# RIVM-bioinformatics/TrueConsense

Measured on NVIDIA B200. Metric: aligned_bases_per_sec_pileup_consensus, higher is better.
Workload: dtype int32

## Files before the change

### trueconsense_b200/csrc/cuda/inserts.cu

```cuda
#include <cub/device/device_segmented_radix_sort.cuh>

#include <memory>
#include <new>

#include "tc_common.cuh"

constexpr int INS_TILE = 256;
constexpr uint64_t KEY_NONE = ~0ull;
constexpr int INS_TBL = 4096;
constexpr int INS_BASES_FIXED = 64;

struct ins_args {
    dreads r;
    const int32_t* cand;
    int n_cand;
    const int32_t* n_cand_dev;
    uint32_t flag_filter; int min_mapq, min_bq, ignore_orphans; long long max_depth;
    int32_t span_hint;
    int32_t* range;
    uint32_t* range_off;
    const int64_t* seg_off;
    const int32_t* tile_cand;
    const int32_t* tile_first;
    int32_t* tile_sel;
    int32_t* tile_last;
    uint64_t* ent_key; int32_t* ent_indel; int32_t* ent_qpos; uint8_t* ent_head;
    uint8_t* ent_sel;
    uint8_t* ent_q;
    uint8_t* pair_q; unsigned long long pair_cap; unsigned long long* pair_bump;
    int olap_mode;
    int32_t* seg_count;
    int32_t* pair_any;
    int32_t* overflow;
    const int32_t* layout;
    uint8_t* bases_fixed;
    tc_status* status;
};

__device__ __forceinline__ int ins_ncand(const ins_args& a) { return a.n_cand_dev ? min(*a.n_cand_dev, a.n_cand) : a.n_cand; }

__global__ void max_span_kernel(dreads r, tc_status* status) {
    int64_t i = (int64_t)blockIdx.x * blockDim.x + threadIdx.x;
    int span = 0;
    if (i < r.n) {
        if (i > 0 && r.pos[i] < r.pos[i - 1]) atomicCAS(&status->err, 0, TC_ERR_UNSORTED);
        for (uint32_t k = r.cigar_off[i]; k < r.cigar_off[i + 1]; ++k) {
            uint32_t c = r.cigar[k];
            if (op_consumes_ref(c & 15u)) span += (int)(c >> 4);
        }
    }
    span = __reduce_max_sync(0xffffffffu, span);
    if ((threadIdx.x & 31) == 0 && span > 0) atomicMax(&status->max_span, span);
}

// ... 1 lines not shown
    int64_t lo = 0, hi = n;
    while (hi > lo) {
        const int64_t step = (hi - lo + 31) / 32;
        const int64_t i = lo + (int64_t)lane * step;
        const bool ge = i >= hi || pos[i] >= v;
        const unsigned m = __ballot_sync(0xffffffffu, ge);
        if (m == 0u) { lo = lo + 31 * step + 1; continue; }
        const int first = __ffs(m) - 1;
        if (first == 0) return (int)lo;
        hi = min(hi, lo + (int64_t)first * step);
        lo = lo + (int64_t)(first - 1) * step + 1;
    }
    return (int)lo;
}

__global__ void cand_range_kernel(ins_args a) {
    const int ci = blockIdx.x * (blockDim.x >> 5) + (threadIdx.x >> 5);
    const int lane = threadIdx.x & 31;
    if (ci >= ins_ncand(a)) return;
    const int c = a.cand[ci] - 1;
    const int ms = max(a.span_hint > 0 ? a.span_hint : a.status->max_span, 1);
    const int lo = warp_lower_bound(a.r.pos, a.r.n, c - ms + 1, lane);
    const int hi = max(lo, warp_lower_bound(a.r.pos, a.r.n, c + 1, lane));
    if (lane == 0) {
        a.range[2 * ci] = lo;
        a.range[2 * ci + 1] = hi;
        a.range_off[4 * ci] = a.r.seq_off[lo]; a.range_off[4 * ci + 1] = a.r.seq_off[hi];
        a.range_off[4 * ci + 2] = a.r.cigar_off[lo]; a.range_off[4 * ci + 3] = a.r.cigar_off[hi];
    }
}

__device__ __forceinline__ uint64_t mix_key(uint64_t h, uint64_t v) {
    h ^= v + 0x9e3779b97f4a7c15ull + (h << 6) + (h >> 2);
    h *= 0xff51afd7ed558ccdull;
    h ^= h >> 33;
    return h;
}

// ... 52 lines not shown
    for (int t = threadIdx.x; t < n_tiles_s; t += blockDim.x) {
        int lo = 0, hi = n_cand - 1;
        while (lo < hi) { const int mid = (lo + hi + 1) >> 1; if (tile_first[mid] <= t) lo = mid; else hi = mid - 1; }
        tile_cand[t] = lo;
    }
}

__global__ void __launch_bounds__(INS_TILE) ins_select_kernel(ins_args a) {
    __shared__ int wlast[INS_TILE / 32];
    const int tile = blockIdx.x;
    if (a.layout && tile >= a.layout[0]) return;
    const int ci = a.tile_cand[tile];
    const int c = a.cand[ci] - 1;
    const int lo = a.range[2 * ci], hi = a.range[2 * ci + 1];
    const int r = lo + (tile - a.tile_first[ci]) * INS_TILE + threadIdx.x;
    bool sel = false, emit = false, proper = false;
    if (r < hi) {
        const int pos = a.r.pos[r];
        if (r > 0 && pos < a.r.pos[r - 1]) atomicCAS(&a.status->err, 0, TC_ERR_UNSORTED);
        const uint32_t fl = a.r.flag[r];
        const bool pass = !(fl & (a.flag_filter | 4u)) && !(a.min_mapq > 0 && a.r.mapq && (int)a.r.mapq[r] < a.min_mapq) &&
                          !(a.ignore_orphans && (fl & 1u) && !(fl & 2u));
        int indel = 0, qpos = 0, qv = 0; char head = 0; uint64_t key = KEY_NONE;
        if (pass) {
            const uint32_t c0 = a.r.cigar_off[r];
            const int n = (int)(a.r.cigar_off[r + 1] - c0);
            const uint32_t* cig = a.r.cigar + c0;
            const bool rev = (fl & 16u) != 0;
            const int lq = a.r.l_seq[r];
            int x = pos, y = 0;
            bool found = false;
            for (int k = 0; k < n; ++k) {
                const uint32_t cc = cig[k]; const uint32_t op = cc & 15u; const int l = (int)(cc >> 4);
                if (!op_consumes_ref(op)) { if (op == OP_I || op == OP_S) y += l; continue; }
                if (c < x + l) {
                    found = true;
                    const bool match = op_is_match(op);
                    qpos = match ? y + (c - x) : y;
                    if (c == x + l - 1) indel = peek_indel(cig, n, k);
                    qv = (qpos < lq) ? (int)a.r.qual[8ull * a.r.seq_off[r] + qpos] : 0;
                    if (qv >= a.min_bq || a.min_bq > 0) {
                        emit = true;
                        if (match) head = (qpos < lq) ? base_char_upper(seq_code(a.r.seq4 + a.r.seq_off[r], qpos), rev) : 'N';
                        else head = (op == OP_N) ? (rev ? '<' : '>') : '*';
                    }
                    break;
                }
                if (op_is_match(op)) y += l;
                x += l;
            }
            sel = found || (x == pos && pos == c);
            if (emit) {
                const read_syms rs = read_syms_of(a, r);
                bool exact = false;
                if (indel <= 8 && indel > -8192) {
                    exact = true;
                    key = (1ull << 62) | ((uint64_t)((uint8_t)head & 127u) << 54) | ((uint64_t)(uint32_t)(indel + 8192) << 40);
                    for (int j = 1; j <= indel; ++j) key |= (uint64_t)rs.sym(qpos + j) << (5 * (j - 1));
                } else if (indel <= 12) {
                    exact = true;
                    key = (3ull << 61) | ((uint64_t)((uint8_t)head & 127u) << 54) | ((uint64_t)(uint32_t)indel << 48);
                    for (int j = 1; j <= indel; ++j) {
                        const uint32_t sy = rs.sym(qpos + j);
                        exact = exact && sy < 16u;
// ... 15 lines not shown
        proper = sel && (fl & 2u);
    }
    if (__syncthreads_or(proper) && threadIdx.x == 0) a.pair_any[ci] = 1;
    const int nsel = __syncthreads_count(sel);
    int last = __reduce_max_sync(0xffffffffu, sel ? r : -1);
    if ((threadIdx.x & 31) == 0) wlast[threadIdx.x >> 5] = last;
    __syncthreads();
    if (threadIdx.x == 0) {
#pragma unroll
        for (int w = 0; w < INS_TILE / 32; ++w) last = max(last, wlast[w]);
        a.tile_sel[tile] = nsel;
        a.tile_last[tile] = last;
    }
}

__global__ void __launch_bounds__(INS_TILE) ins_admit_kernel(ins_args a) {
    __shared__ int wsum[INS_TILE / 32], wlast[INS_TILE / 32];
    __shared__ long long base_s;
    __shared__ int prev_s;
    const int tile = blockIdx.x;
    if (a.layout && tile >= a.layout[0]) return;
    const int ci = a.tile_cand[tile];
    const int lo = a.range[2 * ci], hi = a.range[2 * ci + 1];
    const int t0 = a.tile_first[ci];
    const int lane = threadIdx.x & 31, warp = threadIdx.x >> 5;
    if (warp == 0) {
        long long base = 0; int prev = -1;
        for (int t = t0 + lane; t < tile; t += 32) { base += a.tile_sel[t]; prev = max(prev, a.tile_last[t]); }
#pragma unroll
        for (int o = 16; o; o >>= 1) { base += __shfl_xor_sync(0xffffffffu, base, o); prev = max(prev, __shfl_xor_sync(0xffffffffu, prev, o)); }
// ... 8 lines not shown
#pragma unroll
    for (int o = 1; o < 32; o <<= 1) { const int t = __shfl_up_sync(0xffffffffu, m, o); if (lane >= o) m = max(m, t); }
    int prev = __shfl_up_sync(0xffffffffu, m, 1);
    if (lane == 0) prev = -1;
    if (lane == 31) wlast[warp] = m;
    if (lane == 0) wsum[warp] = __popc(bal);
    __syncthreads();
    long long rank = base_s + __popc(bal & ((1u << lane) - 1));
    prev = max(prev, prev_s);
    for (int w = 0; w < warp; ++w) { rank += wsum[w]; prev = max(prev, wlast[w]); }
    bool admitted = false;
    if (sel) {
        const bool first_at_start = prev < 0 || a.r.pos[prev] != a.r.pos[r];
        admitted = first_at_start || rank < a.max_depth;
    }
    if (a.min_bq > 0) {
        if (r < hi && admitted) a.ent_sel[slot] = (uint8_t)(es | 4);
        return;
    }
    if (emit && !admitted) a.ent_key[slot] = KEY_NONE;
    const int n_adm = __syncthreads_count(emit && admitted);
    if (threadIdx.x == 0 && n_adm) atomicAdd(&a.seg_count[ci], n_adm);
}

__device__ __forceinline__ uint32_t wang_hash(uint32_t key) {
    key += ~(key << 15); key ^= (key >> 10); key += (key << 3); key ^= (key >> 6); key += ~(key << 11); key ^= (key >> 16);
    return key;
}

struct cwalk { const uint32_t* cig; const uint32_t* end; long long icig, iseq, iref; };

__device__ int iref2iseq_set(cwalk& w, long long pos) {
    if (pos < 0) return -1;
    w.icig = 0; w.iseq = 0; w.iref = 0;
    while (w.cig < w.end) {
        const uint32_t cig = *w.cig & 15u; const long long ncig = (long long)(*w.cig >> 4);
        if (cig == OP_S) { w.cig++; w.iseq += ncig; w.icig = 0; continue; }
// ... 98 lines not shown
        for (uint32_t k = a.r.cigar_off[r]; k < a.r.cigar_off[r + 1]; ++k) { const uint32_t c = a.r.cigar[k]; if (op_consumes_ref(c & 15u)) end += (int)(c >> 4); }
        if (mp >= end) return false;
    }
    return true;
}

__global__ void __launch_bounds__(1024) ins_pair_kernel(ins_args a) {
    extern __shared__ __align__(16) unsigned char pair_smem[];
    unsigned int* tmin = reinterpret_cast<unsigned int*>(pair_smem);
    unsigned int* tmax = tmin + PAIR_TBL;
    unsigned short* tcnt = reinterpret_cast<unsigned short*>(tmax + PAIR_TBL);
    __shared__ int over_s, nadm_s;
    const int ci = blockIdx.x;
    if (ci >= ins_ncand(a)) return;
    if (a.layout && a.layout[2]) return;
    const int64_t off = a.seg_off[ci];
    const int lo = a.range[2 * ci];
    const int n = a.range[2 * ci + 1] - lo;
    const bool pairing = a.olap_mode != 1 && a.r.qname_hash && a.r.mpos && a.r.isize && a.pair_any[ci];
    if (threadIdx.x == 0) { over_s = 0; nadm_s = 0; }
    if (pairing) {
        for (int i = threadIdx.x; i < PAIR_TBL; i += blockDim.x) { tmin[i] = 0u; tmax[i] = 0u; tcnt[i] = 0; }
        __syncthreads();
        auto is_event = [&](int i, bool& push) -> bool {
            const uint8_t es = a.ent_sel[off + i];
            if (!(es & 1)) return false;
            if (!(es & 4)) { push = false; return true; }
            push = true;
            return true;
        };
        for (int pass = 0; pass < 2; ++pass) {
            for (int i = threadIdx.x; i < n; i += blockDim.x) {
                bool push;
                if (!is_event(i, push) || push != (pass == 0)) continue;
                const uint32_t r = (uint32_t)(lo + i);
                if (push && !(a.r.flag[r] & 2u)) continue;
                const unsigned long long k = a.r.qname_hash[r];
                unsigned h = (unsigned)(k ^ (k >> 31)) & (PAIR_TBL - 1);
                int probes = 0;
                for (;;) {
                    const unsigned cur = push ? atomicCAS(&tmin[h], 0u, (unsigned)i + 1u) : tmin[h];
                    if (cur == 0u && !push) break;
                    if (cur == 0u || a.r.qname_hash[lo + cur - 1] == k) {
                        atomicMin(&tmin[h], (unsigned)i + 1u); atomicMax(&tmax[h], (unsigned)i + 1u);
                        atomicAdd(reinterpret_cast<unsigned int*>(tcnt) + (h >> 1), (h & 1) ? 0x10000u : 1u);
                        break;
                    }
                    h = (h + 1) & (PAIR_TBL - 1);
                    if (++probes >= PAIR_TBL * 3 / 4) { over_s = 1; break; }
                }
            }
            __syncthreads();
        }
        __syncthreads();
        if (over_s) { if (threadIdx.x == 0) atomicCAS(&a.status->err, 0, TC_ERR_CAPACITY); return; }
        for (int h = threadIdx.x; h < PAIR_TBL; h += blockDim.x) {
            const int cnt = tcnt[h];
            if (cnt < 2) continue;
            const int first = (int)tmin[h] - 1, last = (int)tmax[h] - 1;
            const unsigned long long k = a.r.qname_hash[lo + first];
            int stored = -1;
            int seen = 0;
            for (int i = first; i <= last && seen < cnt; i = (cnt == 2 && i == first) ? last : i + 1) {
                bool push;
                if (!is_event(i, push)) continue;
                const uint32_t r = (uint32_t)(lo + i);
                if (a.r.qname_hash[r] != k || (push && !(a.r.flag[r] & 2u))) continue;
                ++seen;
                if (!push) { stored = -1; continue; }
                if (!olap_eligible(a, r)) continue;
                bool has_span = false;
                for (uint32_t q = a.r.cigar_off[r]; q < a.r.cigar_off[r + 1] && !has_span; ++q) { const uint32_t c = a.r.cigar[q]; has_span = op_consumes_ref(c & 15u) && (c >> 4) > 0; }
                if (!has_span) continue;
                if (stored < 0) {
                    const int mp = a.r.mpos[r];
                    if (mp >= a.r.pos[r] || ((a.r.flag[r] & 1u) && mp == -1)) stored = i;
                    continue;
                }
                const int64_t sa = off + stored, sb = off + i;
                const uint32_t ra = (uint32_t)(lo + stored);
                const int la = a.r.l_seq[ra], lb = a.r.l_seq[r];
                const unsigned long long at = atomicAdd(a.pair_bump, (unsigned long long)(la + lb));
                if (at + (unsigned long long)(la + lb) <= a.pair_cap) {
                    uint8_t* aq = a.pair_q + at; uint8_t* bq = aq + la;
                    const uint8_t* ga = a.r.qual + 8ull * a.r.seq_off[ra]; const uint8_t* gb = a.r.qual + 8ull * a.r.seq_off[r];
                    for (int q = 0; q < la; ++q) aq[q] = ga[q];
                    for (int q = 0; q < lb; ++q) bq[q] = gb[q];
                    tweak_pair(a, ra, r, aq, bq, a.olap_mode);
                    if ((a.ent_sel[sa] & 2) && a.ent_qpos[sa] < la) a.ent_q[sa] = aq[a.ent_qpos[sa]];
                    if ((a.ent_sel[sb] & 2) && a.ent_qpos[sb] < lb) a.ent_q[sb] = bq[a.ent_qpos[sb]];
                } else atomicOr(a.overflow, 2);
                stored = -1;
            }
        }
        __syncthreads();
    }
    int mine = 0;
    for (int i = threadIdx.x; i < n; i += blockDim.x) {
        const uint8_t es = a.ent_sel[off + i];
        const bool ok = (es & 6) == 6 && (int)a.ent_q[off + i] >= a.min_bq;
        if (!ok) a.ent_key[off + i] = KEY_NONE;
        mine += ok ? 1 : 0;
    }
    mine = __reduce_add_sync(0xffffffffu, mine);
    if ((threadIdx.x & 31) == 0 && mine) atomicAdd(&nadm_s, mine);
    __syncthreads();
    if (threadIdx.x == 0) a.seg_count[ci] = nadm_s;
}

__device__ __forceinline__ bool same_entry(const ins_args& a, int lo, int64_t off, uint32_t e1, uint32_t e2) {
    if (a.ent_head[e1] != a.ent_head[e2] || a.ent_indel[e1] != a.ent_indel[e2]) return false;
    const int indel = a.ent_indel[e1];
    if (indel <= 0) return true;
    const read_syms s1 = read_syms_of(a, (uint32_t)(lo + (int64_t)e1 - off)), s2 = read_syms_of(a, (uint32_t)(lo + (int64_t)e2 - off));
    const int q1 = a.ent_qpos[e1], q2 = a.ent_qpos[e2];
    for (int j = 1; j <= indel; ++j)
        if (s1.sym(q1 + j) != s2.sym(q2 + j)) return false;
// ... 15 lines not shown
        const uint32_t e = (uint32_t)off + (uint32_t)(0xffffffffull - (best & 0xffffffffull));
        out.mode_count = (int32_t)(best >> 32);
        out.first_read = (int32_t)(a.range[2 * ci] + (int64_t)e - off);
        out.head = a.ent_head[e];
        out.indel = a.ent_indel[e];
        out.bases_off = (int64_t)e;
        if (out.indel > 0 && out.indel <= INS_BASES_FIXED) {
            const read_syms rs = read_syms_of(a, (uint32_t)out.first_read);
            const int q = a.ent_qpos[e];
            for (int j = 1; j <= out.indel; ++j) a.bases_fixed[(size_t)ci * INS_BASES_FIXED + j - 1] = sym_char(rs.sym(q + j));
        }
    }
    calls[ci] = out;
}

__global__ void __launch_bounds__(1024) ins_count_kernel(ins_args a, tc_insert_call_t* __restrict__ calls) {
    extern __shared__ __align__(16) unsigned char ins_smem[];
    unsigned long long* tkey = reinterpret_cast<unsigned long long*>(ins_smem);
    unsigned int* tcnt = reinterpret_cast<unsigned int*>(tkey + INS_TBL);
    unsigned int* tfirst = tcnt + INS_TBL;
    __shared__ unsigned long long best_s;
    __shared__ int over_s, hashed_s;
    const int ci = blockIdx.x;
    if (ci >= ins_ncand(a)) return;
    if (a.layout && a.layout[2]) return;
    const int64_t off = a.seg_off[ci];
    const int lo = a.range[2 * ci];
    const int n = a.range[2 * ci + 1] - lo;
    for (int i = threadIdx.x; i < INS_TBL; i += blockDim.x) { tkey[i] = KEY_NONE; tcnt[i] = 0; tfirst[i] = 0xffffffffu; }
    if (threadIdx.x == 0) { best_s = 0ull; over_s = 0; hashed_s = 0; }
    __syncthreads();
    for (int base = 0; base < n; base += 4 * (int)blockDim.x) {
        unsigned long long kk[4];
#pragma unroll
        for (int u = 0; u < 4; ++u) {
            const int i = base + u * (int)blockDim.x + (int)threadIdx.x;
            kk[u] = i < n ? a.ent_key[off + i] : KEY_NONE;
        }
#pragma unroll
        for (int u = 0; u < 4; ++u) {
            const int i = base + u * (int)blockDim.x + (int)threadIdx.x;
            const unsigned long long k = kk[u];
            const unsigned grp = __match_any_sync(0xffffffffu, k);
            if (k == KEY_NONE || (__ffs(grp) - 1) != (int)(threadIdx.x & 31)) continue;
            if (!(k >> 62)) hashed_s = 1;
            unsigned h = (unsigned)(k ^ (k >> 29)) & (INS_TBL - 1);
            int probes = 0;
            for (;;) {
                const unsigned long long old = atomicCAS(&tkey[h], KEY_NONE, k);
                if (old == KEY_NONE || old == k) { atomicAdd(&tcnt[h], (unsigned)__popc(grp)); atomicMin(&tfirst[h], (unsigned)i); break; }
                h = (h + 1) & (INS_TBL - 1);
                if (++probes >= INS_TBL * 7 / 8) { over_s = 1; break; }
            }
        }
    }
    __syncthreads();
    if (over_s) { if (threadIdx.x == 0) atomicOr(a.overflow, 1); return; }
    if (hashed_s)
    for (int i = threadIdx.x; i < n; i += blockDim.x) {
        const unsigned long long k = a.ent_key[off + i];
        if (k == KEY_NONE || (k >> 62)) continue;
        unsigned h = (unsigned)(k ^ (k >> 29)) & (INS_TBL - 1);
        while (tkey[h] != k) h = (h + 1) & (INS_TBL - 1);
        const unsigned f = tfirst[h];
        if (f != (unsigned)i && !same_entry(a, lo, off, (uint32_t)(off + f), (uint32_t)(off + i))) atomicCAS(&a.status->err, 0, TC_ERR_RANGE);
    }
    unsigned long long best = 0ull;
    for (int i = threadIdx.x; i < INS_TBL; i += blockDim.x)
        if (tcnt[i]) best = max(best, ((unsigned long long)tcnt[i] << 32) | (0xffffffffull - (unsigned long long)tfirst[i]));
    atomicMax(&best_s, best);
    __syncthreads();
    if (threadIdx.x == 0) write_call(a, ci, a.seg_count[ci], best_s, calls);
}

__global__ void __launch_bounds__(1024) ins_mode_kernel(ins_args a, const uint64_t* __restrict__ skey, const uint32_t* __restrict__ sidx,
                                                        tc_insert_call_t* __restrict__ calls) {
    __shared__ unsigned long long best_s;
    const int ci = blockIdx.x;
    const int64_t off = a.seg_off[ci];
    const int lo_read = a.range[2 * ci];
    const int m = a.seg_count[ci];
    if (threadIdx.x == 0) best_s = 0ull;
    __syncthreads();
    unsigned long long best = 0ull;
    for (int i = threadIdx.x; i < m; i += blockDim.x) {
        const uint64_t k = skey[off + i];
        int lo = 0, hi = i;
// ... 31 lines not shown
    for (int j = threadIdx.x; j < c.indel; j += blockDim.x) bases[c.bases_off + j] = (uint8_t)ins_char(a, r, a.ent_qpos[e], j + 1, rev);
}

static ins_block ins_block_of(int n_cand, bool with_extra) {
    static_assert(sizeof(tc_status) <= 64, "tc_status outgrew its place in the results block");
    ins_block b;
    b.layout = 64; b.over = 80; b.bump = 88;
    b.extra = with_extra ? 128 : 0;
    b.seg = with_extra ? b.extra + 4 * (TC_RB_EXTRA_CAND + (size_t)n_cand) : 96;
    b.calls = b.seg + ((4 * (2 * (size_t)n_cand + 2) + 15) & ~(size_t)15);
    b.fixed = b.calls + sizeof(tc_insert_call_t) * (size_t)n_cand;
    b.bytes = b.fixed + (size_t)n_cand * INS_BASES_FIXED;
    return b;
}

static int ins_bind(tc_ctx* ctx, ins_args& a, uint8_t* d_rb, const ins_block& rb, size_t T, size_t NT, int n_cand, const tc_pileup_params_t* p) {
    const size_t bytes = T * (8 + 4 + 4 + 1 + 1 + 1) + NT * 12 + ((size_t)n_cand + 1) * 16 + 256 + 16;
    uint8_t* slab = (uint8_t*)tc_dev_buf(ctx, SLOT_INS_D, bytes);
    if (!slab) return TC_ERR_NOMEM;
    a.ent_key = (uint64_t*)slab;
    int64_t* d_off = (int64_t*)(a.ent_key + T);
    a.seg_off = d_off;
    a.ent_indel = (int32_t*)(d_off + n_cand + 1); a.ent_qpos = a.ent_indel + T;
    int32_t* d_tcand = a.ent_qpos + T; int32_t* d_tfirst = d_tcand + NT;
    a.tile_cand = d_tcand; a.tile_first = d_tfirst;
    a.tile_sel = d_tfirst + n_cand + 1; a.tile_last = a.tile_sel + NT;
    a.ent_head = (uint8_t*)(a.tile_last + NT); a.ent_sel = a.ent_head + T; a.ent_q = a.ent_sel + T;
    a.seg_count = (int32_t*)(d_rb + rb.seg); a.pair_any = a.seg_count + n_cand + 1; a.overflow = (int32_t*)(d_rb + rb.over);
    a.bases_fixed = d_rb + rb.fixed;
    if (ctx->pair_cap <= 0) ctx->pair_cap = 1 << 22;
    a.pair_bump = (unsigned long long*)(d_rb + rb.bump); a.pair_cap = (unsigned long long)ctx->pair_cap;
    a.pair_q = (uint8_t*)tc_dev_buf(ctx, SLOT_INS_F, (size_t)ctx->pair_cap);
    if (!a.pair_q) return TC_ERR_NOMEM;
    a.flag_filter = p->flag_filter; a.min_mapq = p->min_mapq; a.min_bq = p->min_base_quality; a.ignore_orphans = p->ignore_orphans;
    a.olap_mode = (p->reserved >> 8) & 3;
// ... 16 lines not shown
        ins_select_kernel<<<tiles, INS_TILE, 0, s>>>(a);
        TC_LAUNCH_CHECK();
        ins_admit_kernel<<<tiles, INS_TILE, 0, s>>>(a);
        TC_LAUNCH_CHECK();
    }
    if (a.min_bq > 0) {
        const size_t smem = (size_t)PAIR_TBL * 10;
        if (!(ctx->ins_attr_set & 2)) {
            TC_CUDA(cudaFuncSetAttribute(ins_pair_kernel, cudaFuncAttributeMaxDynamicSharedMemorySize, (int)smem));
            ctx->ins_attr_set |= 2;
        }
        ins_pair_kernel<<<grid, 1024, smem, s>>>(a);
        TC_LAUNCH_CHECK();
    }
    if (d_calls) {
        const size_t smem = (size_t)INS_TBL * 16;
        if (!(ctx->ins_attr_set & 1)) {
            TC_CUDA(cudaFuncSetAttribute(ins_count_kernel, cudaFuncAttributeMaxDynamicSharedMemorySize, (int)smem));
            ctx->ins_attr_set |= 1;
        }
        ins_count_kernel<<<grid, 1024, smem, s>>>(a, d_calls);
        TC_LAUNCH_CHECK();
    }
    return TC_OK;
}

static int ins_check_status(tc_ctx* ctx, const tc_status& st) {
    if (st.err == TC_ERR_UNSORTED) return tc_fail(ctx, TC_ERR_UNSORTED, "Unsorted input. Pileup aborts");
    if (st.err) return tc_fail(ctx, st.err, "insertion key collision or device-side failure %d", st.err);
    return TC_OK;
}

static int ins_place_bases(tc_ctx* ctx, tc_insert_call_t* calls, int n, const uint8_t* fixed, uint8_t* bases, int64_t bases_cap,
                           int64_t* need_out = nullptr) {
    int64_t need = 0;
    for (int i = 0; i < n; ++i) {
// ... 42 lines not shown
    if (!ctx) return TC_ERR_ARG;
    if (!reads || !p || (n_cand > 0 && (!cand_pos || !calls)) || n_cand < 0 || ref_len <= 0) return tc_fail(ctx, TC_ERR_ARG, "bad argument");
    if (n_cand == 0) return TC_OK;
    if (tc_is_device_ptr(cand_pos) || tc_is_device_ptr(calls) || (bases && tc_is_device_ptr(bases)))
        return tc_fail(ctx, TC_ERR_ARG, "tc_extract_inserts takes host pointers for cand_pos / calls / bases");
    for (int i = 0; i < n_cand; ++i)
        if (cand_pos[i] < 1 || cand_pos[i] > ref_len) return tc_fail(ctx, TC_ERR_ARG, "candidate position %d outside 1..%d", cand_pos[i], ref_len);
    cudaStream_t s = (cudaStream_t)stream;
    TC_CUDA(cudaSetDevice(ctx->device));
    auto upload = [&](const void* d, const void* h, size_t bytes, const char* what) {
        const int rc = ins_copy(ctx, d, h, bytes, cudaMemcpyHostToDevice, s, what);
        if (rc == TC_OK) ctx->h2d_bytes += (int64_t)bytes;
        return rc;
    };
    tc_pileup_params_t q = *p;
    for (;;) {
        ins_args a;
        memset(&a, 0, sizeof(a));
        const bool bounded = reads->max_ref_span > 0 && ctx->span_ok_bound == reads->max_ref_span && ctx->span_ok_cigar == reads->cigar &&
                             ctx->span_ok_off == reads->cigar_off && ctx->span_ok_n == reads->n_reads && ctx->span_ok_ops == reads->n_cigar_ops;
        const int stage = NEED_QUAL | NEED_MATE | DEFER_SEQ | DEFER_QUAL | DEFER_MATE | (bounded ? DEFER_CIGAR : 0);
        const bool host_seq = reads->seq4 && !tc_is_device_ptr(reads->seq4);
        const bool host_qual = reads->qual && !tc_is_device_ptr(reads->qual);
        const bool host_cig = bounded && reads->cigar && !tc_is_device_ptr(reads->cigar);
        const bool host_mate = reads->qname_hash && reads->mpos && reads->isize && !tc_is_device_ptr(reads->qname_hash);
        int rc = tc_resolve_reads(ctx, reads, &a.r, stage, s);
        if (rc) return rc;
        const int64_t n = a.r.n;
        for (int i = 0; i < n_cand; ++i) { calls[i].pos = cand_pos[i]; calls[i].n_entries = 0; calls[i].mode_count = 0; calls[i].first_read = -1; calls[i].head = 0; calls[i].indel = 0; calls[i].bases_off = -1; }
        if (n == 0) return TC_OK;
        const ins_block rb = ins_block_of(n_cand, false);
        uint8_t* d_rb = (uint8_t*)tc_dev_buf(ctx, SLOT_INS_E, rb.bytes + 16);
        int32_t* d_cand = (int32_t*)tc_dev_buf(ctx, SLOT_INS_A, 4 * (size_t)n_cand);
        int32_t* d_range = (int32_t*)tc_dev_buf(ctx, SLOT_INS_B, 24 * (size_t)n_cand);
        if (!d_rb || !d_cand || !d_range) return TC_ERR_NOMEM;
        a.status = (tc_status*)d_rb;
        TC_CUDA(cudaMemsetAsync(d_rb, 0, rb.calls, s));
        TC_CUDA(cudaMemcpyAsync(d_cand, cand_pos, 4 * (size_t)n_cand, cudaMemcpyHostToDevice, s));
        ctx->h2d_bytes += 4 * (int64_t)n_cand;
        a.span_hint = bounded ? reads->max_ref_span : 0;
        if (a.span_hint == 0) {
            max_span_kernel<<<(unsigned)((n + 255) / 256), 256, 0, s>>>(a.r, a.status);
            TC_LAUNCH_CHECK();
        }
        a.cand = d_cand; a.n_cand = n_cand; a.range = d_range; a.range_off = (uint32_t*)(d_range + 2 * (size_t)n_cand);
        cand_range_kernel<<<(n_cand + 3) / 4, 128, 0, s>>>(a);
        TC_LAUNCH_CHECK();
        const bool spec = !(host_seq || host_qual || host_cig || host_mate) && q.kernel != 2 && !(q.reserved & 1);
        if (ctx->ins_slot_cap <= 0) ctx->ins_slot_cap = 1 << 16;
        std::unique_ptr<int64_t[]> h_off;
        std::unique_ptr<int32_t[]> h_tfirst, h_tcand;
        int64_t total = ctx->ins_slot_cap;
        int n_tiles = (int)(total / INS_TILE) + n_cand + 1;
        if (!spec) {
            auto h_range = host_array<int32_t>(6 * (size_t)n_cand);
            h_off = host_array<int64_t>((size_t)n_cand + 1);
            h_tfirst = host_array<int32_t>((size_t)n_cand + 1);
            if (!h_range || !h_off || !h_tfirst) return tc_fail(ctx, TC_ERR_NOMEM, "out of host memory");
            if ((rc = ins_copy(ctx, h_range.get(), d_range, 24 * (size_t)n_cand, cudaMemcpyDeviceToHost, s, "range readback")) ||
                (rc = ins_sync(ctx, s, "range readback")))
                return rc;
// ... 18 lines not shown
            if (rc) return rc;
            h_off[0] = 0; h_tfirst[0] = 0;
            for (int i = 0; i < n_cand; ++i) {
                const int64_t len = h_range[2 * i + 1] - h_range[2 * i];
                h_off[i + 1] = h_off[i] + len;
                h_tfirst[i + 1] = h_tfirst[i] + (int32_t)((len + INS_TILE - 1) / INS_TILE);
            }
            total = h_off[n_cand];
            n_tiles = h_tfirst[n_cand];
            if (total >= 0x7fffffffll) return tc_fail(ctx, TC_ERR_CAPACITY, "too many candidate column entries (%lld)", (long long)total);
            h_tcand = host_array<int32_t>((size_t)n_tiles);
            if (!h_tcand) return tc_fail(ctx, TC_ERR_NOMEM, "out of host memory");
            for (int i = 0; i < n_cand; ++i) for (int t = h_tfirst[i]; t < h_tfirst[i + 1]; ++t) h_tcand[t] = i;
        }
        const size_t T = (size_t)(total > 0 ? total : 1), NT = (size_t)(n_tiles > 0 ? n_tiles : 1);
        if ((rc = ins_bind(ctx, a, d_rb, rb, T, NT, n_cand, &q))) return rc;
        tc_insert_call_t* d_calls = (tc_insert_call_t*)(d_rb + rb.calls);
        if (spec) rc = ins_layout_dev(ctx, a, d_rb, rb, T, NT, nullptr, s);
        else if (!(rc = upload(a.seg_off, h_off.get(), 8 * ((size_t)n_cand + 1), "offset upload")) &&
                 !(rc = upload(a.tile_first, h_tfirst.get(), 4 * ((size_t)n_cand + 1), "tile table upload")) && n_tiles)
            rc = upload(a.tile_cand, h_tcand.get(), 4 * (size_t)n_tiles, "tile table upload");
        if (rc) return rc;
        const bool sorted_form = q.kernel == 2;
        if ((rc = ins_enqueue_count(ctx, a, (unsigned)n_tiles, n_cand, sorted_form ? nullptr : d_calls, s))) return rc;
        int32_t h_over = 0;
        unsigned long long h_bump = 0;
        int32_t h_layout[3] = {0, 0, 0};
        const size_t calls_bytes = sizeof(tc_insert_call_t) * (size_t)n_cand, fixed_bytes = (size_t)n_cand * INS_BASES_FIXED;
        auto h_fixed = host_array<uint8_t>(fixed_bytes);
        if (!h_fixed) return tc_fail(ctx, TC_ERR_NOMEM, "out of host memory");
        if (rb.bytes <= TC_HOST_SCRATCH) {
// ... 88 lines not shown
    if (rc) return rc;
    const int64_t n = a.r.n;
    const ins_block rb = ins_block_of(cap, true);
    if (rb.bytes > TC_HOST_SCRATCH) return tc_fail(ctx, TC_ERR_ARG, "candidate capacity %d too large for the pinned results block", cap);
    uint8_t* d_rb = (uint8_t*)tc_dev_buf(ctx, SLOT_INS_E, rb.bytes + 16);
    int32_t* d_range = (int32_t*)tc_dev_buf(ctx, SLOT_INS_B, 24 * (size_t)cap);
    if (!d_rb || !d_range) return TC_ERR_NOMEM;
    TC_CUDA(cudaMemsetAsync(d_rb, 0, rb.calls, s));
    a.span_hint = reads->max_ref_span > 0 ? reads->max_ref_span : 0;
    a.status = (tc_status*)d_rb;
    if (a.span_hint == 0 && n > 0) {
        max_span_kernel<<<(unsigned)((n + 255) / 256), 256, 0, s>>>(a.r, a.status);
        TC_LAUNCH_CHECK();
    }
    a.cand = d_cand; a.n_cand = cap; a.n_cand_dev = d_ncand; a.range = d_range; a.range_off = (uint32_t*)(d_range + 2 * (size_t)cap);
    cand_range_kernel<<<(cap + 3) / 4, 128, 0, s>>>(a);
    TC_LAUNCH_CHECK();
    if (ctx->ins_slot_cap <= 0) ctx->ins_slot_cap = 1 << 16;
    const size_t T = (size_t)ctx->ins_slot_cap, NT = T / INS_TILE + (size_t)cap + 1;
    if ((rc = ins_bind(ctx, a, d_rb, rb, T, NT, cap, p)) || (rc = ins_layout_dev(ctx, a, d_rb, rb, T, NT, d_pileup_status, s))) return rc;
    if (n > 0 && (rc = ins_enqueue_count(ctx, a, (unsigned)NT, cap, (tc_insert_call_t*)(d_rb + rb.calls), s))) return rc;
    TC_CUDA(cudaMemcpyAsync(host_block, d_rb, rb.bytes, cudaMemcpyDeviceToHost, s));
    ctx->d2h_bytes += (int64_t)rb.bytes;
    pend->rb = rb; pend->cap = cap; pend->n_reads = n;
    return TC_OK;
}

int tc_inserts_finish_dev(tc_ctx* ctx, const tc_ins_pending* pend, const void* host_block, tc_status* pileup_status, int32_t* cands, int32_t* n_cand,
                          tc_insert_call_t* calls, uint8_t* bases, int64_t bases_cap, int* fit) {
    const uint8_t* pin = (const uint8_t*)host_block;
    const ins_block& rb = pend->rb;
    const int32_t* extra = (const int32_t*)(pin + rb.extra);
    tc_status st; memcpy(&st, pin, sizeof(st));
    memcpy(pileup_status, extra + TC_RB_EXTRA_STATUS, sizeof(tc_status));
    int32_t layout[3]; memcpy(layout, pin + rb.layout, 12);
// ... 18 lines not shown
```

Baseline: 1231 billion.

## Count insert keys in per-tile shared tables merged into global hash tables

```diff
diff --git a/trueconsense_b200/csrc/cuda/inserts.cu b/trueconsense_b200/csrc/cuda/inserts.cu
--- a/trueconsense_b200/csrc/cuda/inserts.cu
+++ b/trueconsense_b200/csrc/cuda/inserts.cu
@@ -8,7 +8,10 @@
 constexpr int INS_TILE = 256;
 constexpr uint64_t KEY_NONE = ~0ull;
 constexpr int INS_TBL = 4096;
+constexpr int INS_HASH_MAX_CAND = 1024;
 constexpr int INS_BASES_FIXED = 64;
+
+struct __align__(16) ins_slot { unsigned long long key; unsigned int cnt, first; };
 
 struct ins_args {
     dreads r;
@@ -27,6 +30,7 @@
     uint64_t* ent_key; int32_t* ent_indel; int32_t* ent_qpos; uint8_t* ent_head;
     uint8_t* ent_sel;
     uint8_t* ent_q;
+    ins_slot* tbl;
     uint8_t* pair_q; unsigned long long pair_cap; unsigned long long* pair_bump;
     int olap_mode;
     int32_t* seg_count;
@@ -38,6 +42,10 @@
 };
 
 __device__ __forceinline__ int ins_ncand(const ins_args& a) { return a.n_cand_dev ? min(*a.n_cand_dev, a.n_cand) : a.n_cand; }
+
+__device__ __forceinline__ bool ins_pairing(const ins_args& a, int ci) {
+    return a.olap_mode != 1 && a.r.qname_hash && a.r.mpos && a.r.isize && a.pair_any[ci];
+}
 
 __global__ void max_span_kernel(dreads r, tc_status* status) {
     int64_t i = (int64_t)blockIdx.x * blockDim.x + threadIdx.x;
@@ -69,14 +77,22 @@
     return (int)lo;
 }
 
-__global__ void cand_range_kernel(ins_args a) {
-    const int ci = blockIdx.x * (blockDim.x >> 5) + (threadIdx.x >> 5);
-    const int lane = threadIdx.x & 31;
-    if (ci >= ins_ncand(a)) return;
-    const int c = a.cand[ci] - 1;
-    const int ms = max(a.span_hint > 0 ? a.span_hint : a.status->max_span, 1);
-    const int lo = warp_lower_bound(a.r.pos, a.r.n, c - ms + 1, lane);
-    const int hi = max(lo, warp_lower_bound(a.r.pos, a.r.n, c + 1, lane));
+constexpr int RANGE_BLOCK = 128;
+__global__ void __launch_bounds__(RANGE_BLOCK) cand_range_kernel(ins_args a) {
+    __shared__ int bound_s[RANGE_BLOCK / 32];
+    const int warp = threadIdx.x >> 5, lane = threadIdx.x & 31;
+    const int ci = blockIdx.x * (RANGE_BLOCK / 64) + (warp >> 1);
+    const bool live = ci < ins_ncand(a);
+    if (live) {
+        const int c = a.cand[ci] - 1;
+        const int ms = max(a.span_hint > 0 ? a.span_hint : a.status->max_span, 1);
+        const int b = warp_lower_bound(a.r.pos, a.r.n, (warp & 1) ? c + 1 : c - ms + 1, lane);
+        if (lane == 0) bound_s[warp] = b;
+    }
+    __syncthreads();
+    if (!live || (warp & 1)) return;
+    const int lo = bound_s[warp];
+    const int hi = max(lo, bound_s[warp + 1]);
     if (lane == 0) {
         a.range[2 * ci] = lo;
         a.range[2 * ci + 1] = hi;
@@ -159,6 +175,10 @@
     const int c = a.cand[ci] - 1;
     const int lo = a.range[2 * ci], hi = a.range[2 * ci + 1];
     const int r = lo + (tile - a.tile_first[ci]) * INS_TILE + threadIdx.x;
+    if (tile == a.tile_first[ci] && a.tbl) {
+        const ins_slot empty = {KEY_NONE, 0u, 0xffffffffu};
+        for (int h = threadIdx.x; h < INS_TBL; h += INS_TILE) a.tbl[(size_t)ci * INS_TBL + h] = empty;
+    }
     bool sel = false, emit = false, proper = false;
     if (r < hi) {
         const int pos = a.r.pos[r];
@@ -175,24 +195,36 @@
             const int lq = a.r.l_seq[r];
             int x = pos, y = 0;
             bool found = false;
-            for (int k = 0; k < n; ++k) {
-                const uint32_t cc = cig[k]; const uint32_t op = cc & 15u; const int l = (int)(cc >> 4);
-                if (!op_consumes_ref(op)) { if (op == OP_I || op == OP_S) y += l; continue; }
-                if (c < x + l) {
-                    found = true;
-                    const bool match = op_is_match(op);
-                    qpos = match ? y + (c - x) : y;
-                    if (c == x + l - 1) indel = peek_indel(cig, n, k);
-                    qv = (qpos < lq) ? (int)a.r.qual[8ull * a.r.seq_off[r] + qpos] : 0;
-                    if (qv >= a.min_bq || a.min_bq > 0) {
-                        emit = true;
-                        if (match) head = (qpos < lq) ? base_char_upper(seq_code(a.r.seq4 + a.r.seq_off[r], qpos), rev) : 'N';
-                        else head = (op == OP_N) ? (rev ? '<' : '>') : '*';
-                    }
-                    break;
+            const uintptr_t a0 = reinterpret_cast<uintptr_t>(cig);
+            const uint4* cv = reinterpret_cast<const uint4*>(a0 & ~(uintptr_t)15);
+            int kf = -1;
+            uint32_t cf = 0;
+            for (int g = -(int)((a0 & 15) >> 2); g < n && kf < 0; g += 4) {
+                const uint4 v = __ldg(cv++);
+                const uint32_t ops[4] = {v.x, v.y, v.z, v.w};
+#pragma unroll
+                for (int j = 0; j < 4; ++j) {
+                    const int k = g + j;
+                    if (kf >= 0 || k < 0 || k >= n) continue;
+                    const uint32_t cc = ops[j]; const uint32_t op = cc & 15u; const int l = (int)(cc >> 4);
+                    if (!op_consumes_ref(op)) { if (op == OP_I || op == OP_S) y += l; continue; }
+                    if (c < x + l) { kf = k; cf = cc; continue; }
+                    if (op_is_match(op)) y += l;
+                    x += l;
                 }
-                if (op_is_match(op)) y += l;
-                x += l;
+            }
+            if (kf >= 0) {
+                found = true;
+                const uint32_t op = cf & 15u; const int l = (int)(cf >> 4);
+                const bool match = op_is_match(op);
+                qpos = match ? y + (c - x) : y;
+                if (c == x + l - 1) indel = peek_indel(cig, n, kf);
+                qv = (qpos < lq) ? (int)a.r.qual[8ull * a.r.seq_off[r] + qpos] : 0;
+                if (qv >= a.min_bq || a.min_bq > 0) {
+                    emit = true;
+                    if (match) head = (qpos < lq) ? base_char_upper(seq_code(a.r.seq4 + a.r.seq_off[r], qpos), rev) : 'N';
+                    else head = (op == OP_N) ? (rev ? '<' : '>') : '*';
+                }
             }
             sel = found || (x == pos && pos == c);
             if (emit) {
@@ -238,6 +270,47 @@
     }
 }
 
+__device__ __forceinline__ unsigned tbl_slot(unsigned long long k, int size) {
+    return (unsigned)((k * 0x9e3779b97f4a7c15ull) >> (64 - (__ffs(size) - 1)));
+}
+
+__device__ void tbl_add(const ins_args& a, int ci, unsigned long long k, unsigned c, unsigned f) {
+    ins_slot* t = a.tbl + (size_t)ci * INS_TBL;
+    unsigned h = tbl_slot(k, INS_TBL);
+    for (int probes = 0;;) {
+        unsigned long long cur = __ldcg(&t[h].key);
+        if (cur == KEY_NONE) cur = atomicCAS(&t[h].key, KEY_NONE, k);
+        if (cur == KEY_NONE || cur == k) { atomicAdd(&t[h].cnt, c); atomicMin(&t[h].first, f); return; }
+        h = (h + 1) & (INS_TBL - 1);
+        if (++probes >= INS_TBL * 7 / 8) { atomicOr(a.overflow, 1); return; }
+    }
+}
+
+__device__ __forceinline__ void warp_count(const ins_args& a, int ci, unsigned long long k, int i) {
+    const unsigned grp = __match_any_sync(0xffffffffu, k);
+    if (k != KEY_NONE && (__ffs(grp) - 1) == (int)(threadIdx.x & 31)) tbl_add(a, ci, k, (unsigned)__popc(grp), (unsigned)i);
+}
+
+constexpr int INS_TILE_TBL = 2 * INS_TILE;
+__device__ void tile_count(const ins_args& a, int ci, unsigned long long k, int i) {
+    __shared__ unsigned long long skey[INS_TILE_TBL];
+    __shared__ unsigned int scnt[INS_TILE_TBL], sfirst[INS_TILE_TBL];
+    for (int h = threadIdx.x; h < INS_TILE_TBL; h += INS_TILE) { skey[h] = KEY_NONE; scnt[h] = 0u; sfirst[h] = 0xffffffffu; }
+    __syncthreads();
+    const unsigned grp = __match_any_sync(0xffffffffu, k);
+    if (k != KEY_NONE && (__ffs(grp) - 1) == (int)(threadIdx.x & 31)) {
+        unsigned h = tbl_slot(k, INS_TILE_TBL);
+        for (;;) {
+            const unsigned long long cur = atomicCAS(&skey[h], KEY_NONE, k);
+            if (cur == KEY_NONE || cur == k) { atomicAdd(&scnt[h], (unsigned)__popc(grp)); atomicMin(&sfirst[h], (unsigned)i); break; }
+            h = (h + 1) & (INS_TILE_TBL - 1);
+        }
+    }
+    __syncthreads();
+    for (int h = threadIdx.x; h < INS_TILE_TBL; h += INS_TILE)
+        if (scnt[h]) tbl_add(a, ci, skey[h], scnt[h], sfirst[h]);
+}
+
 __global__ void __launch_bounds__(INS_TILE) ins_admit_kernel(ins_args a) {
     __shared__ int wsum[INS_TILE / 32], wlast[INS_TILE / 32];
     __shared__ long long base_s;
@@ -276,13 +349,15 @@
         const bool first_at_start = prev < 0 || a.r.pos[prev] != a.r.pos[r];
         admitted = first_at_start || rank < a.max_depth;
     }
-    if (a.min_bq > 0) {
+    if (a.min_bq > 0 && ins_pairing(a, ci)) {
         if (r < hi && admitted) a.ent_sel[slot] = (uint8_t)(es | 4);
         return;
     }
-    if (emit && !admitted) a.ent_key[slot] = KEY_NONE;
-    const int n_adm = __syncthreads_count(emit && admitted);
+    const bool ok = emit && admitted && (a.min_bq <= 0 || (int)a.ent_q[slot] >= a.min_bq);
+    if (emit && !ok) a.ent_key[slot] = KEY_NONE;
+    const int n_adm = __syncthreads_count(ok);
     if (threadIdx.x == 0 && n_adm) atomicAdd(&a.seg_count[ci], n_adm);
+    if (a.tbl && n_adm) tile_count(a, ci, ok ? a.ent_key[slot] : KEY_NONE, r - lo);
 }
 
 __device__ __forceinline__ uint32_t wang_hash(uint32_t key) {
@@ -411,93 +486,97 @@
     const int ci = blockIdx.x;
     if (ci >= ins_ncand(a)) return;
     if (a.layout && a.layout[2]) return;
+    if (!ins_pairing(a, ci)) return;
     const int64_t off = a.seg_off[ci];
     const int lo = a.range[2 * ci];
     const int n = a.range[2 * ci + 1] - lo;
-    const bool pairing = a.olap_mode != 1 && a.r.qname_hash && a.r.mpos && a.r.isize && a.pair_any[ci];
     if (threadIdx.x == 0) { over_s = 0; nadm_s = 0; }
-    if (pairing) {
-        for (int i = threadIdx.x; i < PAIR_TBL; i += blockDim.x) { tmin[i] = 0u; tmax[i] = 0u; tcnt[i] = 0; }
+    for (int i = threadIdx.x; i < PAIR_TBL; i += blockDim.x) { tmin[i] = 0u; tmax[i] = 0u; tcnt[i] = 0; }
+    __syncthreads();
+    auto is_event = [&](int i, bool& push) -> bool {
+        const uint8_t es = a.ent_sel[off + i];
+        if (!(es & 1)) return false;
+        if (!(es & 4)) { push = false; return true; }
+        push = true;
+        return true;
+    };
+    for (int pass = 0; pass < 2; ++pass) {
+        for (int i = threadIdx.x; i < n; i += blockDim.x) {
+            bool push;
+            if (!is_event(i, push) || push != (pass == 0)) continue;
+            const uint32_t r = (uint32_t)(lo + i);
+            if (push && !(a.r.flag[r] & 2u)) continue;
+            const unsigned long long k = a.r.qname_hash[r];
+            unsigned h = (unsigned)(k ^ (k >> 31)) & (PAIR_TBL - 1);
+            int probes = 0;
+            for (;;) {
+                const unsigned cur = push ? atomicCAS(&tmin[h], 0u, (unsigned)i + 1u) : tmin[h];
+                if (cur == 0u && !push) break;
+                if (cur == 0u || a.r.qname_hash[lo + cur - 1] == k) {
+                    atomicMin(&tmin[h], (unsigned)i + 1u); atomicMax(&tmax[h], (unsigned)i + 1u);
+                    atomicAdd(reinterpret_cast<unsigned int*>(tcnt) + (h >> 1), (h & 1) ? 0x10000u : 1u);
+                    break;
+                }
+                h = (h + 1) & (PAIR_TBL - 1);
+                if (++probes >= PAIR_TBL * 3 / 4) { over_s = 1; break; }
+            }
+        }
         __syncthreads();
-        auto is_event = [&](int i, bool& push) -> bool {
+    }
+    __syncthreads();
+    if (over_s) { if (threadIdx.x == 0) atomicCAS(&a.status->err, 0, TC_ERR_CAPACITY); return; }
+    for (int h = threadIdx.x; h < PAIR_TBL; h += blockDim.x) {
+        const int cnt = tcnt[h];
+        if (cnt < 2) continue;
+        const int first = (int)tmin[h] - 1, last = (int)tmax[h] - 1;
+        const unsigned long long k = a.r.qname_hash[lo + first];
+        int stored = -1;
+        int seen = 0;
+        for (int i = first; i <= last && seen < cnt; i = (cnt == 2 && i == first) ? last : i + 1) {
+            bool push;
+            if (!is_event(i, push)) continue;
+            const uint32_t r = (uint32_t)(lo + i);
+            if (a.r.qname_hash[r] != k || (push && !(a.r.flag[r] & 2u))) continue;
+            ++seen;
+            if (!push) { stored = -1; continue; }
+            if (!olap_eligible(a, r)) continue;
+            bool has_span = false;
+            for (uint32_t q = a.r.cigar_off[r]; q < a.r.cigar_off[r + 1] && !has_span; ++q) { const uint32_t c = a.r.cigar[q]; has_span = op_consumes_ref(c & 15u) && (c >> 4) > 0; }
+            if (!has_span) continue;
+            if (stored < 0) {
+                const int mp = a.r.mpos[r];
+                if (mp >= a.r.pos[r] || ((a.r.flag[r] & 1u) && mp == -1)) stored = i;
+                continue;
+            }
+            const int64_t sa = off + stored, sb = off + i;
+            const uint32_t ra = (uint32_t)(lo + stored);
+            const int la = a.r.l_seq[ra], lb = a.r.l_seq[r];
+            const unsigned long long at = atomicAdd(a.pair_bump, (unsigned long long)(la + lb));
+            if (at + (unsigned long long)(la + lb) <= a.pair_cap) {
+                uint8_t* aq = a.pair_q + at; uint8_t* bq = aq + la;
+                const uint8_t* ga = a.r.qual + 8ull * a.r.seq_off[ra]; const uint8_t* gb = a.r.qual + 8ull * a.r.seq_off[r];
+                for (int q = 0; q < la; ++q) aq[q] = ga[q];
+                for (int q = 0; q < lb; ++q) bq[q] = gb[q];
+                tweak_pair(a, ra, r, aq, bq, a.olap_mode);
+                if ((a.ent_sel[sa] & 2) && a.ent_qpos[sa] < la) a.ent_q[sa] = aq[a.ent_qpos[sa]];
+                if ((a.ent_sel[sb] & 2) && a.ent_qpos[sb] < lb) a.ent_q[sb] = bq[a.ent_qpos[sb]];
+            } else atomicOr(a.overflow, 2);
+            stored = -1;
+        }
+    }
+    __syncthreads();
+    int mine = 0;
+    for (int base = 0; base < n; base += blockDim.x) {
+        const int i = base + (int)threadIdx.x;
+        unsigned long long k = KEY_NONE;
+        if (i < n) {
             const uint8_t es = a.ent_sel[off + i];
-            if (!(es & 1)) return false;
-            if (!(es & 4)) { push = false; return true; }
-            push = true;
-            return true;
-        };
-        for (int pass = 0; pass < 2; ++pass) {
-            for (int i = threadIdx.x; i < n; i += blockDim.x) {
-                bool push;
-                if (!is_event(i, push) || push != (pass == 0)) continue;
-                const uint32_t r = (uint32_t)(lo + i);
-                if (push && !(a.r.flag[r] & 2u)) continue;
-                const unsigned long long k = a.r.qname_hash[r];
-                unsigned h = (unsigned)(k ^ (k >> 31)) & (PAIR_TBL - 1);
-                int probes = 0;
-                for (;;) {
-                    const unsigned cur = push ? atomicCAS(&tmin[h], 0u, (unsigned)i + 1u) : tmin[h];
-                    if (cur == 0u && !push) break;
-                    if (cur == 0u || a.r.qname_hash[lo + cur - 1] == k) {
-                        atomicMin(&tmin[h], (unsigned)i + 1u); atomicMax(&tmax[h], (unsigned)i + 1u);
-                        atomicAdd(reinterpret_cast<unsigned int*>(tcnt) + (h >> 1), (h & 1) ? 0x10000u : 1u);
-                        break;
-                    }
-                    h = (h + 1) & (PAIR_TBL - 1);
-                    if (++probes >= PAIR_TBL * 3 / 4) { over_s = 1; break; }
-                }
-            }
-            __syncthreads();
-        }
-        __syncthreads();
-        if (over_s) { if (threadIdx.x == 0) atomicCAS(&a.status->err, 0, TC_ERR_CAPACITY); return; }
-        for (int h = threadIdx.x; h < PAIR_TBL; h += blockDim.x) {
-            const int cnt = tcnt[h];
-            if (cnt < 2) continue;
-            const int first = (int)tmin[h] - 1, last = (int)tmax[h] - 1;
-            const unsigned long long k = a.r.qname_hash[lo + first];
-            int stored = -1;
-            int seen = 0;
-            for (int i = first; i <= last && seen < cnt; i = (cnt == 2 && i == first) ? last : i + 1) {
-                bool push;
-                if (!is_event(i, push)) continue;
-                const uint32_t r = (uint32_t)(lo + i);
-                if (a.r.qname_hash[r] != k || (push && !(a.r.flag[r] & 2u))) continue;
-                ++seen;
-                if (!push) { stored = -1; continue; }
-                if (!olap_eligible(a, r)) continue;
-                bool has_span = false;
-                for (uint32_t q = a.r.cigar_off[r]; q < a.r.cigar_off[r + 1] && !has_span; ++q) { const uint32_t c = a.r.cigar[q]; has_span = op_consumes_ref(c & 15u) && (c >> 4) > 0; }
-                if (!has_span) continue;
-                if (stored < 0) {
-                    const int mp = a.r.mpos[r];
-                    if (mp >= a.r.pos[r] || ((a.r.flag[r] & 1u) && mp == -1)) stored = i;
-                    continue;
-                }
-                const int64_t sa = off + stored, sb = off + i;
-                const uint32_t ra = (uint32_t)(lo + stored);
-                const int la = a.r.l_seq[ra], lb = a.r.l_seq[r];
-                const unsigned long long at = atomicAdd(a.pair_bump, (unsigned long long)(la + lb));
-                if (at + (unsigned long long)(la + lb) <= a.pair_cap) {
-                    uint8_t* aq = a.pair_q + at; uint8_t* bq = aq + la;
-                    const uint8_t* ga = a.r.qual + 8ull * a.r.seq_off[ra]; const uint8_t* gb = a.r.qual + 8ull * a.r.seq_off[r];
-                    for (int q = 0; q < la; ++q) aq[q] = ga[q];
-                    for (int q = 0; q < lb; ++q) bq[q] = gb[q];
-                    tweak_pair(a, ra, r, aq, bq, a.olap_mode);
-                    if ((a.ent_sel[sa] & 2) && a.ent_qpos[sa] < la) a.ent_q[sa] = aq[a.ent_qpos[sa]];
-                    if ((a.ent_sel[sb] & 2) && a.ent_qpos[sb] < lb) a.ent_q[sb] = bq[a.ent_qpos[sb]];
-                } else atomicOr(a.overflow, 2);
-                stored = -1;
-            }
-        }
-        __syncthreads();
-    }
-    int mine = 0;
-    for (int i = threadIdx.x; i < n; i += blockDim.x) {
-        const uint8_t es = a.ent_sel[off + i];
-        const bool ok = (es & 6) == 6 && (int)a.ent_q[off + i] >= a.min_bq;
-        if (!ok) a.ent_key[off + i] = KEY_NONE;
-        mine += ok ? 1 : 0;
+            const bool ok = (es & 6) == 6 && (int)a.ent_q[off + i] >= a.min_bq;
+            if (!ok) a.ent_key[off + i] = KEY_NONE;
+            else k = a.ent_key[off + i];
+            mine += ok ? 1 : 0;
+        }
+        if (a.tbl) warp_count(a, ci, k, i);
     }
     mine = __reduce_add_sync(0xffffffffu, mine);
     if ((threadIdx.x & 31) == 0 && mine) atomicAdd(&nadm_s, mine);
@@ -543,63 +622,43 @@
     calls[ci] = out;
 }
 
-__global__ void __launch_bounds__(1024) ins_count_kernel(ins_args a, tc_insert_call_t* __restrict__ calls) {
-    extern __shared__ __align__(16) unsigned char ins_smem[];
-    unsigned long long* tkey = reinterpret_cast<unsigned long long*>(ins_smem);
-    unsigned int* tcnt = reinterpret_cast<unsigned int*>(tkey + INS_TBL);
-    unsigned int* tfirst = tcnt + INS_TBL;
+__global__ void __launch_bounds__(1024) ins_pick_kernel(ins_args a, tc_insert_call_t* __restrict__ calls) {
     __shared__ unsigned long long best_s;
-    __shared__ int over_s, hashed_s;
     const int ci = blockIdx.x;
     if (ci >= ins_ncand(a)) return;
     if (a.layout && a.layout[2]) return;
-    const int64_t off = a.seg_off[ci];
-    const int lo = a.range[2 * ci];
-    const int n = a.range[2 * ci + 1] - lo;
-    for (int i = threadIdx.x; i < INS_TBL; i += blockDim.x) { tkey[i] = KEY_NONE; tcnt[i] = 0; tfirst[i] = 0xffffffffu; }
-    if (threadIdx.x == 0) { best_s = 0ull; over_s = 0; hashed_s = 0; }
-    __syncthreads();
-    for (int base = 0; base < n; base += 4 * (int)blockDim.x) {
-        unsigned long long kk[4];
-#pragma unroll
-        for (int u = 0; u < 4; ++u) {
-            const int i = base + u * (int)blockDim.x + (int)threadIdx.x;
-            kk[u] = i < n ? a.ent_key[off + i] : KEY_NONE;
-        }
-#pragma unroll
-        for (int u = 0; u < 4; ++u) {
-            const int i = base + u * (int)blockDim.x + (int)threadIdx.x;
-            const unsigned long long k = kk[u];
-            const unsigned grp = __match_any_sync(0xffffffffu, k);
-            if (k == KEY_NONE || (__ffs(grp) - 1) != (int)(threadIdx.x & 31)) continue;
-            if (!(k >> 62)) hashed_s = 1;
-            unsigned h = (unsigned)(k ^ (k >> 29)) & (INS_TBL - 1);
-            int probes = 0;
-            for (;;) {
-                const unsigned long long old = atomicCAS(&tkey[h], KEY_NONE, k);
-                if (old == KEY_NONE || old == k) { atomicAdd(&tcnt[h], (unsigned)__popc(grp)); atomicMin(&tfirst[h], (unsigned)i); break; }
-                h = (h + 1) & (INS_TBL - 1);
-                if (++probes >= INS_TBL * 7 / 8) { over_s = 1; break; }
-            }
-        }
-    }
-    __syncthreads();
-    if (over_s) { if (threadIdx.x == 0) atomicOr(a.overflow, 1); return; }
-    if (hashed_s)
-    for (int i = threadIdx.x; i < n; i += blockDim.x) {
-        const unsigned long long k = a.ent_key[off + i];
-        if (k == KEY_NONE || (k >> 62)) continue;
-        unsigned h = (unsigned)(k ^ (k >> 29)) & (INS_TBL - 1);
-        while (tkey[h] != k) h = (h + 1) & (INS_TBL - 1);
-        const unsigned f = tfirst[h];
-        if (f != (unsigned)i && !same_entry(a, lo, off, (uint32_t)(off + f), (uint32_t)(off + i))) atomicCAS(&a.status->err, 0, TC_ERR_RANGE);
-    }
+    if (*a.overflow & 1) return;
+    const int m = a.seg_count[ci];
+    if (m == 0) {
+        if (threadIdx.x == 0) write_call(a, ci, 0, 0ull, calls);
+        return;
+    }
+    const ins_slot* t = a.tbl + (size_t)ci * INS_TBL;
+    if (threadIdx.x == 0) best_s = 0ull;
     unsigned long long best = 0ull;
-    for (int i = threadIdx.x; i < INS_TBL; i += blockDim.x)
-        if (tcnt[i]) best = max(best, ((unsigned long long)tcnt[i] << 32) | (0xffffffffull - (unsigned long long)tfirst[i]));
+    bool hashed = false;
+    for (int h = threadIdx.x; h < INS_TBL; h += blockDim.x) {
+        const ins_slot e = t[h];
+        if (!e.cnt) continue;
+        best = max(best, ((unsigned long long)e.cnt << 32) | (0xffffffffull - (unsigned long long)e.first));
+        hashed = hashed || !(e.key >> 62);
+    }
+    if (__syncthreads_or(hashed)) {
+        const int64_t off = a.seg_off[ci];
+        const int lo = a.range[2 * ci];
+        const int n = a.range[2 * ci + 1] - lo;
+        for (int i = threadIdx.x; i < n; i += blockDim.x) {
+            const unsigned long long k = a.ent_key[off + i];
+            if (k == KEY_NONE || (k >> 62)) continue;
+            unsigned h = tbl_slot(k, INS_TBL);
+            while (t[h].key != k) h = (h + 1) & (INS_TBL - 1);
+            const unsigned f = t[h].first;
+            if (f != (unsigned)i && !same_entry(a, lo, off, (uint32_t)(off + f), (uint32_t)(off + i))) atomicCAS(&a.status->err, 0, TC_ERR_RANGE);
+        }
+    }
     atomicMax(&best_s, best);
     __syncthreads();
-    if (threadIdx.x == 0) write_call(a, ci, a.seg_count[ci], best_s, calls);
+    if (threadIdx.x == 0) write_call(a, ci, m, best_s, calls);
 }
 
 __global__ void __launch_bounds__(1024) ins_mode_kernel(ins_args a, const uint64_t* __restrict__ skey, const uint32_t* __restrict__ sidx,
@@ -661,11 +720,14 @@
     return b;
 }
 
-static int ins_bind(tc_ctx* ctx, ins_args& a, uint8_t* d_rb, const ins_block& rb, size_t T, size_t NT, int n_cand, const tc_pileup_params_t* p) {
-    const size_t bytes = T * (8 + 4 + 4 + 1 + 1 + 1) + NT * 12 + ((size_t)n_cand + 1) * 16 + 256 + 16;
+static int ins_bind(tc_ctx* ctx, ins_args& a, uint8_t* d_rb, const ins_block& rb, size_t T, size_t NT, int n_cand, const tc_pileup_params_t* p,
+                    bool tables) {
+    const size_t tbl_bytes = tables ? (size_t)n_cand * INS_TBL * sizeof(ins_slot) : 0;
+    const size_t bytes = tbl_bytes + T * (8 + 4 + 4 + 1 + 1 + 1) + NT * 12 + ((size_t)n_cand + 1) * 16 + 256 + 16;
     uint8_t* slab = (uint8_t*)tc_dev_buf(ctx, SLOT_INS_D, bytes);
     if (!slab) return TC_ERR_NOMEM;
-    a.ent_key = (uint64_t*)slab;
+    a.tbl = tables ? (ins_slot*)slab : nullptr;
+    a.ent_key = (uint64_t*)(slab + tbl_bytes);
     int64_t* d_off = (int64_t*)(a.ent_key + T);
     a.seg_off = d_off;
     a.ent_indel = (int32_t*)(d_off + n_cand + 1); a.ent_qpos = a.ent_indel + T;
@@ -712,12 +774,7 @@
         TC_LAUNCH_CHECK();
     }
     if (d_calls) {
-        const size_t smem = (size_t)INS_TBL * 16;
-        if (!(ctx->ins_attr_set & 1)) {
-            TC_CUDA(cudaFuncSetAttribute(ins_count_kernel, cudaFuncAttributeMaxDynamicSharedMemorySize, (int)smem));
-            ctx->ins_attr_set |= 1;
-        }
-        ins_count_kernel<<<grid, 1024, smem, s>>>(a, d_calls);
+        ins_pick_kernel<<<grid, 1024, 0, s>>>(a, d_calls);
         TC_LAUNCH_CHECK();
     }
     return TC_OK;
@@ -790,6 +847,7 @@
         return rc;
     };
     tc_pileup_params_t q = *p;
+    if (n_cand > INS_HASH_MAX_CAND) q.kernel = 2;
     for (;;) {
         ins_args a;
         memset(&a, 0, sizeof(a));
@@ -820,7 +878,7 @@
             TC_LAUNCH_CHECK();
         }
         a.cand = d_cand; a.n_cand = n_cand; a.range = d_range; a.range_off = (uint32_t*)(d_range + 2 * (size_t)n_cand);
-        cand_range_kernel<<<(n_cand + 3) / 4, 128, 0, s>>>(a);
+        cand_range_kernel<<<(n_cand + RANGE_BLOCK / 64 - 1) / (RANGE_BLOCK / 64), RANGE_BLOCK, 0, s>>>(a);
         TC_LAUNCH_CHECK();
         const bool spec = !(host_seq || host_qual || host_cig || host_mate) && q.kernel != 2 && !(q.reserved & 1);
         if (ctx->ins_slot_cap <= 0) ctx->ins_slot_cap = 1 << 16;
@@ -869,7 +927,7 @@
             for (int i = 0; i < n_cand; ++i) for (int t = h_tfirst[i]; t < h_tfirst[i + 1]; ++t) h_tcand[t] = i;
         }
         const size_t T = (size_t)(total > 0 ? total : 1), NT = (size_t)(n_tiles > 0 ? n_tiles : 1);
-        if ((rc = ins_bind(ctx, a, d_rb, rb, T, NT, n_cand, &q))) return rc;
+        if ((rc = ins_bind(ctx, a, d_rb, rb, T, NT, n_cand, &q, q.kernel != 2))) return rc;
         tc_insert_call_t* d_calls = (tc_insert_call_t*)(d_rb + rb.calls);
         if (spec) rc = ins_layout_dev(ctx, a, d_rb, rb, T, NT, nullptr, s);
         else if (!(rc = upload(a.seg_off, h_off.get(), 8 * ((size_t)n_cand + 1), "offset upload")) &&
@@ -988,11 +1046,11 @@
         TC_LAUNCH_CHECK();
     }
     a.cand = d_cand; a.n_cand = cap; a.n_cand_dev = d_ncand; a.range = d_range; a.range_off = (uint32_t*)(d_range + 2 * (size_t)cap);
-    cand_range_kernel<<<(cap + 3) / 4, 128, 0, s>>>(a);
+    cand_range_kernel<<<(cap + RANGE_BLOCK / 64 - 1) / (RANGE_BLOCK / 64), RANGE_BLOCK, 0, s>>>(a);
     TC_LAUNCH_CHECK();
     if (ctx->ins_slot_cap <= 0) ctx->ins_slot_cap = 1 << 16;
     const size_t T = (size_t)ctx->ins_slot_cap, NT = T / INS_TILE + (size_t)cap + 1;
-    if ((rc = ins_bind(ctx, a, d_rb, rb, T, NT, cap, p)) || (rc = ins_layout_dev(ctx, a, d_rb, rb, T, NT, d_pileup_status, s))) return rc;
+    if ((rc = ins_bind(ctx, a, d_rb, rb, T, NT, cap, p, true)) || (rc = ins_layout_dev(ctx, a, d_rb, rb, T, NT, d_pileup_status, s))) return rc;
     if (n > 0 && (rc = ins_enqueue_count(ctx, a, (unsigned)NT, cap, (tc_insert_call_t*)(d_rb + rb.calls), s))) return rc;
     TC_CUDA(cudaMemcpyAsync(host_block, d_rb, rb.bytes, cudaMemcpyDeviceToHost, s));
     ctx->d2h_bytes += (int64_t)rb.bytes;
```

Result: faster. 1316 billion, median of 6 (+6.9%).
